# Eddie-Wang1120/Eddie-Wang-Hackathon2023

Hardware: AMD Instinct MI355X
Metric: decode tokens/s, whole job (encoder + cross-KV + language-ID + prefill + greedy decode), Whisper large-v2 int8 weight-only + int8 KV; rtf reported beside it (higher is better)
Workload: dtype f16

## Files before the change

### eddie-wang-hackathon2023_amd/csrc/attn_decode.hip

```cpp
#include <hip/hip_ext.h>

#include <atomic>

#include "common.h"
#include "kernels.h"

namespace wm {

constexpr float ATTN_SCALE = 0.35355339059327373f;
constexpr int MAX_L = 4;

template <bool I8>
__global__ __launch_bounds__(64) void attn_self_kernel(AttnSelfParams p) {
    __builtin_amdgcn_s_setprio(3);

    constexpr int MAXT = 512;
    __shared__ float s_p[MAXT];
    __shared__ h16 s_qall[MAX_L][64], s_knew[MAX_L][64], s_vnew[MAX_L][64];

    const int h = blockIdx.x, lane = threadIdx.x;
    int b = blockIdx.y;
    const int32_t* lsrc = p.live ? p.live : (const int32_t*)p.part;
    const int32_t live_n = lsrc[0], live_b = lsrc[p.live ? 1 + b : 0];
    const int32_t t_now = (p.t_dev ? p.t_dev : (const int32_t*)p.part)[0];
// ... 131 lines not shown
            sum += e;
        }
        sum = wave_sum_nomfma(sum);
        const float inv = 1.0f / sum;
        __syncthreads();
        for (int j = lane; j < nk; j += 64) s_p[j] = r16(s_p[j] * inv);
        __syncthreads();
        float o = 0.f;
        int j = 0;
        if (I8) {
            const int8_t* pv = (const int8_t*)pastV + lane;
#pragma unroll
            for (int u = 0; u < 32; ++u)
                if (u < T) o = fmaf(s_p[u], r16((float)vpre8[u] * t_dq), o);
            j = min(T, 32);
            for (; j + 32 <= T; j += 32) {
                int8_t vq[32];
#pragma unroll
                for (int u = 0; u < 32; ++u) vq[u] = pv[(size_t)(j + u) * 64];
#pragma unroll
                for (int u = 0; u < 32; ++u) o = fmaf(s_p[j + u], r16((float)vq[u] * t_dq), o);
            }
            for (; j + 8 <= T; j += 8) {
                int8_t vq[8];
#pragma unroll
                for (int u = 0; u < 8; ++u) vq[u] = pv[(size_t)(j + u) * 64];
#pragma unroll
                for (int u = 0; u < 8; ++u) o = fmaf(s_p[j + u], r16((float)vq[u] * t_dq), o);
            }
            for (; j < T; ++j) o = fmaf(s_p[j], r16((float)pv[(size_t)j * 64] * t_dq), o);
        } else {
            const h16* pv = (const h16*)pastV + lane;
#pragma unroll
            for (int u = 0; u < 32; ++u)
                if (u < T) o = fmaf(s_p[u], (float)vpre16[u], o);
            j = min(T, 32);
            for (; j + 32 <= T; j += 32) {
                h16 vh[32];
#pragma unroll
                for (int u = 0; u < 32; ++u) vh[u] = pv[(size_t)(j + u) * 64];
#pragma unroll
                for (int u = 0; u < 32; ++u) o = fmaf(s_p[j + u], (float)vh[u], o);
            }
            for (; j + 8 <= T; j += 8) {
                h16 vh[8];
#pragma unroll
                for (int u = 0; u < 8; ++u) vh[u] = pv[(size_t)(j + u) * 64];
#pragma unroll
                for (int u = 0; u < 8; ++u) o = fmaf(s_p[j + u], (float)vh[u], o);
            }
            for (; j < T; ++j) o = fmaf(s_p[j], (float)pv[(size_t)j * 64], o);
        }
        for (; j < nk; ++j) o = fmaf(s_p[j], (float)s_vnew[j - T][lane], o);
        p.out[(size_t)(b * p.L + i) * p.ldo + h * 64 + lane] = (h16)f32_as_is(o);
        __syncthreads();
    }
}

constexpr int SELF_WAVES = 4;
template <bool I8>
__global__ __launch_bounds__(64 * SELF_WAVES) void attn_self_wg_kernel(AttnSelfParams p) {
    __builtin_amdgcn_s_setprio(3);
    constexpr int MAXT = 512;
    constexpr int ES = I8 ? 1 : 2;
    constexpr int ROW_B = 64 * ES;
    constexpr int DIMS = 16 / ES;
    constexpr int NCH = 64 / DIMS;
    constexpr int VROWS = 64 / NCH;
    constexpr int KCH = ROW_B / 16;
    constexpr int VPRE = 4;
    constexpr int NT = 64 * SELF_WAVES;
    __shared__ float s_p[MAXT];
    __shared__ h16 s_qall[MAX_L][64], s_knew[MAX_L][64], s_vnew[MAX_L][64];
    __shared__ float s_o[NT][DIMS + 1];
    __shared__ float s_red[2][SELF_WAVES];
    __shared__ float s_lut[I8 ? 512 + MAX_L * 64 : 1];

    const int h = blockIdx.x, tid = threadIdx.x, lane = tid & 63, wid = tid >> 6;
    int b = blockIdx.y;
    const int32_t* lsrc = p.live ? p.live : (const int32_t*)p.part;
    const int32_t live_n = lsrc[0], live_b = lsrc[p.live ? 1 + b : 0];
    const int32_t t_now = (p.t_dev ? p.t_dev : (const int32_t*)p.part)[0];
    if (p.live) {
        if (b >= live_n) return;
        b = live_b;
    }
    const int T = p.t_dev ? t_now : p.T;
    const int C = p.H * 64;
    const unsigned char* pastK = (const unsigned char*)p.past + ((size_t)b * p.past_bstride + (size_t)(0 * p.H + h) * p.past_cap * 64) * ES;
    const unsigned char* pastV = (const unsigned char*)p.past + ((size_t)b * p.past_bstride + (size_t)(1 * p.H + h) * p.past_cap * 64) * ES;
    const int vr = lane / NCH, vc = lane % NCH;
    uint4 kpre[KCH], vpre[VPRE];
    if (T > 0) {
        const int kr = min(64 * wid + lane, T - 1);
#pragma unroll
        for (int c = 0; c < KCH; ++c) kpre[c] = ((const uint4*)(pastK + (size_t)kr * ROW_B))[c];
#pragma unroll
        for (int n = 0; n < VPRE; ++n) {
            const int row = min((wid + SELF_WAVES * n) * VROWS + vr, T - 1);
            vpre[n] = *(const uint4*)(pastV + (size_t)row * ROW_B + vc * 16);
        }
    }
    const float t_dq = p.kv_scale;
    const float inv_t = 1.0f / p.kv_scale;
    if constexpr (I8) {
        const float d = r16((float)(int)(int8_t)(tid & 255) * t_dq);
// ... 104 lines not shown
        __syncthreads();
        const float inv = 1.0f / ((s_red[1][0] + s_red[1][1]) + (s_red[1][2] + s_red[1][3]));
        if (tid < nk) s_p[tid] = r16(e0 * inv);
        if (tid + NT < nk) s_p[tid + NT] = r16(e1 * inv);
        __syncthreads();
        float o[DIMS];
#pragma unroll
        for (int d = 0; d < DIMS; ++d) o[d] = 0.f;
        auto add_block = [&](int vb, const uint4& w) {
            const int row = vb * VROWS + vr;
            const float pj = row < T ? s_p[row] : 0.f;
            if (I8) {
                const uint32_t ws[4] = {w.x, w.y, w.z, w.w};
#pragma unroll
                for (int d = 0; d < 16; ++d)
                    o[d] = fmaf(pj, s_lut[256 + ((ws[d >> 2] >> (8 * (d & 3))) & 0xff)], o[d]);
            } else {
                const half8v wh = __builtin_bit_cast(half8v, w);
#pragma unroll
                for (int d = 0; d < 8; ++d) o[d] = fmaf(pj, (float)wh[d], o[d]);
            }
        };
#pragma unroll
        for (int n = 0; n < VPRE; ++n) {
            const int vb = wid + SELF_WAVES * n;
            if (vb * VROWS < T) add_block(vb, vpre[n]);
        }
        for (int vb = wid + SELF_WAVES * VPRE; vb * VROWS < T; vb += SELF_WAVES) {
            const int row = min(vb * VROWS + vr, T - 1);
            add_block(vb, *(const uint4*)(pastV + (size_t)row * ROW_B + vc * 16));
        }
#pragma unroll
        for (int d = 0; d < DIMS; ++d) s_o[tid][d] = o[d];
        __syncthreads();
        if (wid == 0) {
            const int ch = lane / DIMS, d = lane % DIMS;
            float part[SELF_WAVES][VROWS];
#pragma unroll
            for (int w = 0; w < SELF_WAVES; ++w)
#pragma unroll
                for (int r = 0; r < VROWS; ++r) part[w][r] = s_o[w * 64 + r * NCH + ch][d];
            float acc = 0.f;
#pragma unroll
            for (int w = 0; w < SELF_WAVES; ++w)
#pragma unroll
                for (int r = 0; r < VROWS; ++r) acc += part[w][r];
            for (int j = T; j < nk; ++j) acc = fmaf(s_p[j], (float)s_vnew[j - T][lane], acc);
            p.out[(size_t)(b * p.L + i) * p.ldo + h * 64 + lane] = (h16)f32_as_is(acc);
        }
        __syncthreads();
    }
}

int launch_attn_self(const AttnSelfParams& p, hipStream_t stream) {
    WM_REQUIRE(p.L >= 1 && p.L <= MAX_L, "attn_self: L=%d out of range [1,%d]", p.L, MAX_L);
    WM_REQUIRE(p.T + p.L <= 512, "attn_self: T+L=%d exceeds 512", p.T + p.L);
    WM_REQUIRE(p.T + p.L <= p.present_cap, "attn_self: present capacity %d < T+L=%d", p.present_cap, p.T + p.L);
    WM_REQUIRE(!p.int8_kv || p.kv_scale > 0.f, "attn_self: int8 KV needs a positive scale");
    WM_REQUIRE(p.waves == 0 || p.waves == 1 || p.waves == SELF_WAVES, "attn_self: waves=%d (0, 1 or %d)", p.waves, SELF_WAVES);
    if (p.waves == SELF_WAVES) {
        if (p.int8_kv) hipLaunchKernelGGL(attn_self_wg_kernel<true>, dim3(p.H, p.B), dim3(64 * SELF_WAVES), 0, stream, p);
        else hipLaunchKernelGGL(attn_self_wg_kernel<false>, dim3(p.H, p.B), dim3(64 * SELF_WAVES), 0, stream, p);
    } else if (p.int8_kv)
        hipLaunchKernelGGL(attn_self_kernel<true>, dim3(p.H, p.B), dim3(64), 0, stream, p);
    else
        hipLaunchKernelGGL(attn_self_kernel<false>, dim3(p.H, p.B), dim3(64), 0, stream, p);
    WM_LAUNCH_CHECK(stream, "attn_self");
    return 0;
}

constexpr int CROSS_MAX_KEYS = 1536;
constexpr int CROSS_MAX_SPLIT = 16;


template <int L, bool I8 = false, int UNR_ = 0, bool SKIP = false>
__global__ __launch_bounds__(256) void attn_cross_kernel(AttnCrossParams p) {
    constexpr int DPL = I8 ? 16 : 8;
    constexpr int LPR = 64 / DPL;
    constexpr int RPI = 64 / LPR;
    constexpr int ESZ = I8 ? 1 : 2;
#ifndef CROSS_UNR
#define CROSS_UNR 4
#endif
    constexpr int UNR = UNR_ > 0 ? UNR_ : CROSS_UNR;
    __shared__ float s_sc[L][CROSS_MAX_KEYS];
    __shared__ float s_red[L][4][2];
    __shared__ float s_o[4][L][64];
    __shared__ unsigned char s_live[SKIP ? CROSS_MAX_KEYS / 8 : 1];

    const int tid = threadIdx.x, lane = tid & 63, wid = __builtin_amdgcn_readfirstlane(tid >> 6);
    const int sub = lane % LPR, rowi = lane / LPR;
    const int per_split = (((p.Tk + p.nsplit - 1) / p.nsplit) + 7) & ~7;
    constexpr int STRIDE = 4 * RPI * UNR;
    const int first = wid * (RPI * UNR);
    const int n_rows = p.live ? p.live[0] : p.B;
    const int n_items = p.H * n_rows * p.nsplit;

    struct Item { int h, b, sp, k_begin, nkeys; const unsigned char* K; const unsigned char* V; };
    auto geometry = [&](int item) {
        Item it;
        it.h = item % p.H; it.b = (item / p.H) % n_rows; it.sp = item / (p.H * n_rows);
        if (p.live) it.b = p.live[1 + it.b];
        it.k_begin = it.sp * per_split;
        it.nkeys = max(0, min(p.Tk, it.k_begin + per_split) - it.k_begin);
        it.K = (const unsigned char*)p.kv + ((size_t)it.b * p.kv_bstride + ((size_t)(0 * p.H + it.h) * p.Tk) * 64) * ESZ;
        it.V = (const unsigned char*)p.kv + ((size_t)it.b * p.kv_bstride + ((size_t)(1 * p.H + it.h) * p.Tk) * 64) * ESZ;
        return it;
    };
    auto issue = [&](u32x4 (&dst)[UNR], const unsigned char* base, int k_begin, int nkeys, int r0) {
#pragma unroll
        for (int u = 0; u < UNR; ++u) {
            const int rr = min(r0 + u * RPI + rowi, nkeys - 1);
            dst[u] = __builtin_nontemporal_load((const u32x4*)(base + ((size_t)(k_begin + rr) * 64 + sub * DPL) * ESZ));
        }
        __builtin_amdgcn_sched_barrier(0);
// ... 395 lines not shown
```

### eddie-wang-hackathon2023_amd/csrc/engine.hip

```cpp
#include <stdarg.h>
#include <stdio.h>
#include <stdlib.h>
#include <string.h>

#include <atomic>
#include <map>
#include <mutex>
#include <unordered_map>
#include <string>
#include <vector>

#include "../../include/whisper_mi355.h"
#include "common.h"
#include "kernels.h"

namespace wm {

static thread_local char g_err[1024] = "";
void set_error(const char* fmt, ...) {
    va_list ap;
    va_start(ap, fmt);
    vsnprintf(g_err, sizeof(g_err), fmt, ap);
    va_end(ap);
}
// ... 1229 lines not shown
}

int wm_argmax(const void* logits, int64_t row_stride, int batch, int n_vocab, int32_t* ids, wm_stream_t stream) {
    WM_REQUIRE(logits && ids && batch >= 1 && n_vocab >= 1, "wm_argmax: null argument or empty input");
    return launch_argmax((const h16*)logits, (long)row_stride, batch, n_vocab, ids, (hipStream_t)stream);
}

int wm_gemm_skinny(const void* A, int lda, int M, int K, const void* Wt, int n_blocks, int w8,
                   const void* scale, int ksplit, float* part, wm_stream_t stream) {
    GemmSkinnyParams p{};
    p.A = (const h16*)A; p.lda = lda; p.M = M; p.K = K; p.Wt = Wt; p.n_blocks = n_blocks; p.w8 = w8;
    p.scale = (const h16*)scale; p.ksplit = ksplit; p.part = part;
    return launch_gemm_skinny(p, (hipStream_t)stream);
}
int wm_gemm_skinny_default_ksplit(int M, int K, int n_blocks, int w8) { return skinny_default_ksplit(M, K, n_blocks, w8); }

int wm_set_rows_path(int min_rows) {
    const int prev = rows_path_min_rows();
    g_rows_min.store(min_rows < 0 ? 0 : min_rows, std::memory_order_relaxed);
    return prev;
}

int wm_gemm_rows(const wm_gemv_io* io, wm_stream_t stream) {
    WM_REQUIRE(io && io->a && io->wt, "wm_gemm_rows: null argument");
    GemvSmallParams p{};
    p.A = (const h16*)io->a; p.lda = io->lda; p.M = io->m; p.K = io->k; p.Wt = io->wt; p.n_blocks = io->n_blocks; p.w8 = io->w8;
    p.scale = (const h16*)io->scale;
    p.ln_g = (const h16*)io->ln_gamma; p.ln_b = (const h16*)io->ln_beta;
    p.mode = io->mode; p.bias = (const h16*)io->bias; p.gelu_kind = io->gelu_kind;
    p.out32 = io->out32; p.ld32 = io->ld32; p.out16 = (h16*)io->out16; p.ld16 = io->ld16; p.n_valid = io->n_valid;
    p.x = (h16*)io->x; p.ldx = io->ldx;
    return launch_gemm_rows(p, (hipStream_t)stream);
}

int wm_lab_knobs(char* buf, size_t cap) {
    std::lock_guard<std::mutex> lk(g_lab_mu);
    if (buf && cap > 0) { strncpy(buf, g_lab_honoured.c_str(), cap - 1); buf[cap - 1] = 0; }
    return (int)g_lab_honoured.size();
}

int wm_set_gemm_small_tiles(int tiles) {
    const int prev = get_gemm_small_tiles();
    set_gemm_small_tiles(tiles);
    return prev;
}

int wm_set_self_attn_waves(int waves) {
    self_attn_waves(1);
    const int prev = g_self_waves.load(std::memory_order_relaxed);
    g_self_waves.store(waves == 1 || waves == 4 ? waves : 0, std::memory_order_relaxed);
    return prev;
}

int wm_set_small_batch_rows(int rows) {
    const int prev = small_path_max_rows();
    g_small_rows.store(rows < 0 ? 0 : (rows > GEMV_SMALL_MAX_M ? GEMV_SMALL_MAX_M : rows), std::memory_order_relaxed);
    return prev;
}

int wm_gemv_fused(const wm_gemv_io* io, wm_stream_t stream) {
    WM_REQUIRE(io && io->a && io->wt, "wm_gemv_fused: null argument");
    GemvSmallParams p{};
    p.A = (const h16*)io->a; p.lda = io->lda; p.M = io->m; p.K = io->k; p.Wt = io->wt; p.n_blocks = io->n_blocks; p.w8 = io->w8;
    p.scale = (const h16*)io->scale;
    p.ln_g = (const h16*)io->ln_gamma; p.ln_b = (const h16*)io->ln_beta;
    p.mode = io->mode; p.bias = (const h16*)io->bias; p.gelu_kind = io->gelu_kind;
    p.out32 = io->out32; p.ld32 = io->ld32; p.out16 = (h16*)io->out16; p.ld16 = io->ld16; p.n_valid = io->n_valid;
    p.x = (h16*)io->x; p.ldx = io->ldx;
    return launch_gemv_small(p, (hipStream_t)stream);
}

int wm_layernorm(const void* x, int ldx, int M, int N, const void* gamma, const void* beta, void* out, int ldo,
                 wm_stream_t stream) {
    return launch_layernorm((const h16*)x, ldx, M, N, (const h16*)gamma, (const h16*)beta, (h16*)out, ldo, (hipStream_t)stream);
}

int wm_attn_encoder(const void* qkv, int ld, int B, int T, int H, void* out, int ldo, wm_stream_t stream) {
    AttnEncParams p{(const h16*)qkv, ld, B, T, H, (h16*)out, ldo};
    return launch_attn_encoder(p, (hipStream_t)stream);
}

int wm_attn_decode_cross(const float* q, int B, int L, int H, int Tk, const void* kv, void* out, int nsplit,
                         float* ws, wm_stream_t stream) {
    AttnCrossParams p{};
    p.part = q; p.ksplit = 1; p.ldp = H * 64; p.bias = nullptr;
    p.B = B; p.L = L; p.H = H; p.Tk = Tk; p.kv = (const h16*)kv; p.kv_bstride = (long)2 * H * Tk * 64;
    p.out = (h16*)out; p.ldo = H * 64; p.nsplit = nsplit; p.ws = ws;
    p.skip_zero_rows = g_cross_v_skip.load(std::memory_order_relaxed);
    return launch_attn_cross(p, (hipStream_t)stream);
}

int wm_set_decode_chain(int on) {
    const int prev = g_decode_chain.load(std::memory_order_relaxed);
    g_decode_chain.store(on < 0 ? DECODE_CHAIN_DEFAULT : (on > 2 ? 2 : on), std::memory_order_relaxed);
    for (ChainDev& cd : g_chain_dev) {
        std::lock_guard<std::mutex> lk(cd.mu);
        if (cd.declined) { cd.declined = false; cd.reason.clear(); }
    }
    return prev;
}

int wm_decode_chain_error(int* out) {
    WM_REQUIRE(out, "wm_decode_chain_error: null argument");
    ChainDev& cd = chain_dev_slot(current_device_index());
    const unsigned v = chain_err_peek(cd);
    *out = (int)v;
// ... 5 lines not shown
    }
    return 0;
}

int wm_decode_chain_status(wm_chain_status* out) {
    WM_REQUIRE(out, "wm_decode_chain_status: null argument");
    ChainDev& cd = chain_dev_slot(current_device_index());
    std::lock_guard<std::mutex> lk(cd.mu);
    memset(out, 0, sizeof(*out));
    out->mode = g_decode_chain.load(std::memory_order_relaxed);
    out->launches = cd.launches.load(std::memory_order_relaxed);
    out->declined_calls = cd.declined_calls.load(std::memory_order_relaxed);
    out->declined = cd.declined ? 1 : 0;
    out->error_pending = chain_err_peek(cd) ? 1 : 0;
    snprintf(out->reason, sizeof(out->reason), "%s", cd.reason.c_str());
    snprintf(out->footprint, sizeof(out->footprint), "%s", cd.footprint.c_str());
    return 0;
}

int wm_debug_occupy(int n_workgroups, size_t lds_bytes, int64_t microseconds, wm_stream_t stream) {
    return launch_occupy(n_workgroups, lds_bytes, (long long)microseconds, (hipStream_t)stream);
}

int wm_set_cross_v_skip(int on) {
    const int prev = g_cross_v_skip.load(std::memory_order_relaxed);
    g_cross_v_skip.store(on < 0 ? CROSS_V_SKIP_DEFAULT : (on ? 1 : 0), std::memory_order_relaxed);
    return prev;
}

int wm_attn_decode_cross_i8(const float* q, int B, int L, int H, int Tk, const void* kv_i8, float kv_scale, void* out, int nsplit,
                            float* ws, wm_stream_t stream) {
    WM_REQUIRE(kv_scale > 0.f, "wm_attn_decode_cross_i8: the scale must be positive");
    AttnCrossParams p{};
    p.part = q; p.ksplit = 1; p.ldp = H * 64; p.bias = nullptr;
    p.B = B; p.L = L; p.H = H; p.Tk = Tk; p.kv = (const h16*)kv_i8; p.kv_bstride = (long)2 * H * Tk * 64;
    p.kv_q8_scale = kv_scale;
    p.out = (h16*)out; p.ldo = H * 64; p.nsplit = nsplit; p.ws = ws;
    return launch_attn_cross(p, (hipStream_t)stream);
}

int wm_attn_decode_self(const float* qkv, int B, int L, int T, int H, const void* past, int past_cap,
                        void* present, int present_cap, int int8_kv, float kv_scale, void* out, wm_stream_t stream) {
    AttnSelfParams p{};
    p.part = qkv; p.ksplit = 1; p.ldp = 3 * H * 64; p.bias = nullptr;
    p.B = B; p.L = L; p.T = T; p.H = H;
    p.present = present; p.present_cap = present_cap; p.present_bstride = (long)2 * H * present_cap * 64;
    if (T > 0 && past) { p.past = past; p.past_cap = past_cap; p.past_bstride = (long)2 * H * past_cap * 64; }
    else { p.past = present; p.past_cap = present_cap; p.past_bstride = p.present_bstride; }
    p.int8_kv = int8_kv; p.kv_scale = kv_scale; p.out = (h16*)out; p.ldo = H * 64;
    p.waves = self_attn_waves(B * L);
    return launch_attn_self(p, (hipStream_t)stream);
}

int wm_quantize_i8(const void* x, void* q, int64_t n, float inv_scale, wm_stream_t stream) {
    return launch_quantize_i8((const h16*)x, (int8_t*)q, (long)n, inv_scale, (hipStream_t)stream);
}

size_t wm_log_mel_workspace_bytes(int batch, int n_samples, int n_mels) {
    return log_mel_workspace_bytes(batch, n_samples, n_mels);
}

int wm_log_mel(const float* audio, int batch, int n_samples, int64_t audio_ld, const float* filters, int n_mels,
               void* mel_f16, float* mel_f32, void* workspace, size_t workspace_bytes, wm_stream_t stream) {
    return launch_log_mel(audio, batch, n_samples, (long)audio_ld, filters, n_mels, (h16*)mel_f16, mel_f32, workspace,
                          workspace_bytes, (hipStream_t)stream);
}

}
```

### eddie-wang-hackathon2023_amd/csrc/kernels.h

```cpp
#pragma once
#include "common.h"

namespace wm {

struct GemmBigParams {
    const h16* A; int lda; int M; int K;
    const void* W; int N;
    const h16* bias;
    h16* C; int ldc;
    const h16* residual; int ldr; int res_mod;
    int act;
    int colscale_n; float colscale;
    int out_mode;
    int hs_T, hs_H, hs_kv;
    float q8_inv_scale;
    int a_rows; long a_bstride;
    int c_rows; long c_bstride;
    int max_wgs;
    int nt_flags;
    int tile_rows;
};
int launch_gemm_f16(const GemmBigParams& p, hipStream_t stream);
constexpr int GEMM_SMALL_TILES_DEFAULT = 150;
constexpr int GEMM_TINY_TILES_DEFAULT = 160;
// ... 74 lines not shown
    const float* part; int ksplit; int M; int N; int ldp;
    long part_sstride;
    const h16* bias;
    int mode; int gelu_kind;
    h16* x; int ldx;
    const h16* ln_g; const h16* ln_b;
    h16* out; int ldo;
    int eager;
};
int launch_row_finish(const RowFinishParams& p, hipStream_t stream);

struct EmbedParams {
    const int32_t* tokens; int tokens_ld;
    int M;
    int L;
    const void* emb_tiles; int C;
    const h16* pos;
    h16* x; int ldx;
    int n_vocab;
    const int32_t* t_dev;
    unsigned* generation;
};
int launch_embed(const EmbedParams& p, hipStream_t stream);

int launch_mel_transpose_pad(const h16* mel, int B, int n_mels, int T, h16* out ,
                             hipStream_t stream);
int launch_zero_pad_rows(h16* buf, int B, int Tpad, int C, hipStream_t stream);
int launch_layernorm(const h16* x, int ldx, int M, int N, const h16* g, const h16* b, h16* out, int ldo,
                     hipStream_t stream);

struct AttnEncParams {
    const h16* qkv; int ld;
    int B, T, H;
    h16* out; int ldo;
    int max_wgs;
};
int launch_attn_encoder(const AttnEncParams& p, hipStream_t stream);

struct AttnSelfParams {
    const float* part; int ksplit; int ldp;
    long part_sstride;
    const h16* bias;
    int B, L, T, H;
    const void* past; long past_bstride; int past_cap;
    void* present; long present_bstride; int present_cap;
    int int8_kv; float kv_scale;
    float* amax;
    const int32_t* t_dev;
    h16* out; int ldo;
    const int32_t* live;
    int waves;
};
int launch_attn_self(const AttnSelfParams& p, hipStream_t stream);

struct AttnCrossParams {
    const float* part; int ksplit; int ldp;
    long part_sstride;
    const h16* bias;
    int B, L, H, Tk;
    const h16* kv; long kv_bstride;
    float kv_q8_scale;
    h16* out; int ldo;
    int nsplit;
    float* ws;
    const int32_t* live;
    int skip_zero_rows;
};
constexpr int CROSS_V_SKIP_DEFAULT = 1;
int launch_attn_cross(const AttnCrossParams& p, hipStream_t stream, hipEvent_t ev_start = nullptr, hipEvent_t ev_stop = nullptr);

struct GreedyParams {
    h16* logits; long ld_row;
    int B; int V;
    int32_t* tokens; int ld_tok; int cur_len;
    float* sum_logprobs;
    const int32_t* suppress; int n_suppress;
    const int32_t* blank; int n_blank;
    int sample_begin; int eot; int timestamp_begin; int max_initial_ts;
    int apply_rules;
    int32_t* n_done;
    const int32_t* t_dev;
    int32_t* done;
    const int32_t* row_limit;
    float temperature;
    uint32_t seed_lo, seed_hi; const uint32_t* seed_dev;
    int row0;
};
int launch_greedy(const GreedyParams& p, hipStream_t stream);
int launch_step_advance(int32_t* counter, hipStream_t stream);
int launch_step_finish(int32_t* counter, const int32_t* done, int B, int32_t* live, hipStream_t stream);
int launch_argmax(const h16* logits, long ld_row, int B, int V, int32_t* ids, hipStream_t stream);

constexpr int BEAM_MAX = 8, BEAM_POOL_MAX = 16;
struct BeamCand { float lp; int32_t tok; };
struct BeamParams {
    GreedyParams g;
    int K, max_cand, ignore_eot;
    int32_t* parent;
    int32_t* fin_tokens; float* fin_scores; int32_t* fin_len; int32_t* fin_count;
    int32_t* live_len;
    BeamCand* cand;
};
int launch_beam_step(const BeamParams& p, hipStream_t stream);
struct KvReorderParams {
    void* const* layers; int n_layer, rows, K, H, cap, elem_bytes;
    const int32_t* parent; const int32_t* done; int n_last; const int32_t* t_dev;
// ... 11 lines not shown
```

### eddie-wang-hackathon2023_amd/native.py

```python
from __future__ import annotations

import atexit
import ctypes as C
import os
from typing import Optional, Sequence

import sys
import warnings


def _hip_already_initialised() -> bool:
    t = sys.modules.get("torch")
    try:
        return bool(t is not None and t.cuda.is_initialized())
    except Exception:
        return False


def _configure_runtime() -> dict:
    name = "DEBUG_CLR_GRAPH_PACKET_CAPTURE"
    late = _hip_already_initialised()
    if name in os.environ:
        return {"name": name, "value": os.environ[name], "set_by": "caller", "in_time": None}
    if os.environ.get("WM_GRAPH_NODE_REPLAY", "1") == "0":
        return {"name": name, "value": None, "set_by": "nobody (WM_GRAPH_NODE_REPLAY=0)", "in_time": None}
    os.environ[name] = "0"
    if late:
        warnings.warn("whisper_mi355: the HIP runtime was initialised before this package was imported, so "
                      f"{name}=0 (node-by-node graph replay, 6-10 % of the small-batch token step) is NOT in effect: "
                      "import the package before the first torch.cuda call, or export the variable yourself", RuntimeWarning, stacklevel=3)
    return {"name": name, "value": "0", "set_by": "package", "in_time": not late}


RUNTIME_KNOBS = _configure_runtime()


def runtime_report() -> dict:
    rep = dict(RUNTIME_KNOBS)
    rep["effective_env"] = os.environ.get(RUNTIME_KNOBS["name"])
    if _lib is not None:
        buf = C.create_string_buffer(4096)
        _lib.wm_lab_knobs(buf, 4096)
        rep["lab_knobs_honoured"] = buf.value.decode() or None
    return rep


_HERE = os.path.dirname(os.path.abspath(__file__))
LIB_PATH = os.environ.get("WM_LIBRARY_PATH") or os.path.join(_HERE, "libwhisper_mi355.so")

EXPORTS = (
    "wm_version", "wm_last_error", "wm_device_count", "wm_engine_create", "wm_engine_destroy",
    "wm_engine_info", "wm_engine_weight_bytes", "wm_encoder_workspace_bytes", "wm_encoder_forward",
    "wm_encoder_forward_shared", "wm_encoder_forward_range",
    "wm_cross_kv_workspace_bytes", "wm_cross_kv", "wm_decoder_workspace_bytes", "wm_decoder_step",
    "wm_greedy_step", "wm_gemm", "wm_gemm_skinny", "wm_gemm_skinny_default_ksplit", "wm_layernorm",
    "wm_attn_encoder", "wm_attn_decode_cross", "wm_attn_decode_self", "wm_quantize_i8",
    "wm_profile_configure", "wm_profile_read", "wm_step_advance", "wm_log_mel_workspace_bytes", "wm_log_mel",
    "wm_flac_info", "wm_flac_decode", "wm_conv1d_gelu", "wm_argmax", "wm_gemv_fused", "wm_gemm_rows", "wm_set_rows_path", "wm_set_small_batch_rows", "wm_set_self_attn_waves", "wm_set_gemm_small_tiles", "wm_lab_knobs", "wm_set_cross_v_skip", "wm_set_decode_chain", "wm_decode_chain_error", "wm_decode_chain_status", "wm_debug_occupy", "wm_decoder_step_multi", "wm_stream_create_cu_mask", "wm_stream_destroy", "wm_attn_decode_cross_i8", "wm_debug_timeline",
    "wm_step_finish",
    "wm_beam_workspace_bytes", "wm_beam_step", "wm_kv_reorder",
    "wm_gemm_ex", "wm_row_finish", "wm_embed", "wm_mel_transpose_pad", "wm_zero_pad_rows",
)


ABI_VERSION = 8

import threading as _threading
CAPTURE_LOCK = _threading.RLock()


class WmError(RuntimeError):
    pass


class WmFlacStreamInfo(C.Structure):
    _fields_ = [("sample_rate", C.c_int32), ("channels", C.c_int32), ("bits_per_sample", C.c_int32),
                ("max_block_size", C.c_int32), ("total_samples", C.c_int64), ("md5", C.c_uint8 * 16)]


class WmChainStatus(C.Structure):
    _fields_ = [("mode", C.c_int32), ("declined", C.c_int32), ("error_pending", C.c_int32), ("pad_", C.c_int32),
                ("launches", C.c_int64), ("declined_calls", C.c_int64), ("reason", C.c_char * 200), ("footprint", C.c_char * 200)]


def chain_status() -> dict:
    st = WmChainStatus()
    check(load_library().wm_decode_chain_status(C.byref(st)), "wm_decode_chain_status")
    return {"mode": st.mode, "declined": bool(st.declined), "error_pending": bool(st.error_pending), "launches": int(st.launches),
            "declined_calls": int(st.declined_calls), "reason": st.reason.decode(), "footprint": st.footprint.decode()}


class WmDims(C.Structure):
    _fields_ = [(n, C.c_int32) for n in (
        "n_mels", "n_audio_ctx", "n_audio_state", "n_audio_head", "n_audio_layer",
        "n_vocab", "n_text_ctx", "n_text_state", "n_text_head", "n_text_layer")]

    def to_dict(self):
        return {n: int(getattr(self, n)) for n, _ in self._fields_}


class WmDecoderIO(C.Structure):
    _fields_ = [
        ("batch", C.c_int32), ("n_new", C.c_int32), ("n_past", C.c_int32),
        ("tokens", C.c_void_p), ("tokens_ld", C.c_int32), ("positional_embedding", C.c_void_p),
        ("past", C.POINTER(C.c_void_p)), ("past_capacity", C.c_int32),
        ("present", C.POINTER(C.c_void_p)), ("present_capacity", C.c_int32),
        ("cross", C.POINTER(C.c_void_p)),
        ("logits", C.c_void_p),
        ("workspace", C.c_void_p), ("workspace_bytes", C.c_size_t),
        ("qkv_amax", C.c_void_p),
        ("n_past_dev", C.c_void_p),
# ... 84 lines not shown
        ("x", C.c_void_p), ("ldx", C.c_int32),
        ("ln_gamma", C.c_void_p), ("ln_beta", C.c_void_p),
        ("out", C.c_void_p), ("ldo", C.c_int32),
    ]


_lib: Optional[C.CDLL] = None


def load_library(path: str = LIB_PATH) -> C.CDLL:
    global _lib
    if _lib is not None:
        return _lib
    if not os.path.exists(path):
        raise WmError(f"{path} not found: build it with `python __graft_entry__.py` "
                      f"(hipcc --offload-arch=gfx950); there is no fallback path")
    lib = C.CDLL(path, mode=C.RTLD_GLOBAL)
    for name in EXPORTS:
        if not hasattr(lib, name):
            raise WmError(f"{path} does not export {name}")
    vp, i32, sz = C.c_void_p, C.c_int, C.c_size_t
    lib.wm_version.restype = i32
    if lib.wm_version() != ABI_VERSION:
        raise WmError(f"{path} has ABI version {lib.wm_version()}, this binding needs {ABI_VERSION}: rebuild it "
                      f"(python __graft_entry__.py)")
    lib.wm_last_error.restype = C.c_char_p
    lib.wm_device_count.argtypes = [C.POINTER(i32)]
    lib.wm_engine_create.argtypes = [vp, sz, i32, C.POINTER(vp)]
    lib.wm_engine_destroy.argtypes = [vp]
    lib.wm_engine_destroy.restype = None
    lib.wm_engine_info.argtypes = [vp, C.POINTER(C.c_int32), C.POINTER(C.c_uint32), C.POINTER(WmDims)]
    lib.wm_engine_weight_bytes.argtypes = [vp]
    lib.wm_engine_weight_bytes.restype = sz
    lib.wm_encoder_workspace_bytes.argtypes = [vp, i32]
    lib.wm_encoder_workspace_bytes.restype = sz
    lib.wm_encoder_forward.argtypes = [vp, vp, i32, vp, vp, sz, vp]
    lib.wm_encoder_forward_shared.argtypes = [vp, vp, i32, vp, vp, sz, i32, vp]
    lib.wm_encoder_forward_range.argtypes = [vp, vp, i32, vp, vp, sz, i32, i32, i32, vp]
    lib.wm_cross_kv_workspace_bytes.argtypes = [vp, i32]
    lib.wm_cross_kv_workspace_bytes.restype = sz
    lib.wm_cross_kv.argtypes = [vp, vp, i32, C.POINTER(vp), vp, sz, vp]
    lib.wm_decoder_workspace_bytes.argtypes = [vp, i32, i32]
    lib.wm_decoder_workspace_bytes.restype = sz
    lib.wm_decoder_step.argtypes = [vp, C.POINTER(WmDecoderIO), vp]
    lib.wm_greedy_step.argtypes = [C.POINTER(WmGreedyIO), vp]
    lib.wm_gemm.argtypes = [vp, i32, i32, i32, vp, i32, i32, vp, vp, vp, i32, i32, vp, i32, vp, sz, vp]
    lib.wm_conv1d_gelu.argtypes = [vp, i32, i32, i32, vp, i32, vp, i32, i32, i32, vp, vp]
    lib.wm_argmax.argtypes = [vp, C.c_int64, i32, i32, vp, vp]
    lib.wm_gemv_fused.argtypes = [C.POINTER(WmGemvIO), vp]
    lib.wm_set_small_batch_rows.argtypes = [i32]
    lib.wm_gemm_rows.argtypes = [C.POINTER(WmGemvIO), vp]
    lib.wm_set_rows_path.argtypes = [i32]
    lib.wm_set_self_attn_waves.argtypes = [i32]
    lib.wm_set_gemm_small_tiles.argtypes = [i32]
    lib.wm_lab_knobs.argtypes = [C.c_char_p, sz]
    lib.wm_set_cross_v_skip.argtypes = [i32]
    lib.wm_set_decode_chain.argtypes = [i32]
    lib.wm_decode_chain_error.argtypes = [C.POINTER(C.c_int)]
    lib.wm_decode_chain_status.argtypes = [C.POINTER(WmChainStatus)]
    lib.wm_debug_occupy.argtypes = [i32, sz, C.c_int64, vp]
    lib.wm_gemm_skinny.argtypes = [vp, i32, i32, i32, vp, i32, i32, vp, i32, vp, vp]
    lib.wm_gemm_skinny_default_ksplit.argtypes = [i32, i32, i32, i32]
    lib.wm_layernorm.argtypes = [vp, i32, i32, i32, vp, vp, vp, i32, vp]
    lib.wm_attn_encoder.argtypes = [vp, i32, i32, i32, i32, vp, i32, vp]
    lib.wm_attn_decode_cross.argtypes = [vp, i32, i32, i32, i32, vp, vp, i32, vp, vp]
    lib.wm_attn_decode_self.argtypes = [vp, i32, i32, i32, i32, vp, i32, vp, i32, i32, C.c_float, vp, vp]
    lib.wm_quantize_i8.argtypes = [vp, vp, C.c_int64, C.c_float, vp]
    lib.wm_log_mel_workspace_bytes.argtypes = [i32, i32, i32]
    lib.wm_log_mel_workspace_bytes.restype = sz
    lib.wm_log_mel.argtypes = [vp, i32, i32, C.c_int64, vp, i32, vp, vp, vp, sz, vp]
    lib.wm_decoder_step_multi.argtypes = [vp, i32, C.POINTER(C.POINTER(WmDecoderIO)), C.POINTER(vp), vp]
    lib.wm_stream_create_cu_mask.argtypes = [C.POINTER(C.c_uint32), i32, C.POINTER(vp)]
    lib.wm_stream_destroy.argtypes = [vp]
    lib.wm_attn_decode_cross_i8.argtypes = [vp, i32, i32, i32, i32, vp, C.c_float, vp, i32, vp, vp]
    lib.wm_flac_info.argtypes = [vp, sz, C.POINTER(WmFlacStreamInfo)]
    lib.wm_flac_decode.argtypes = [vp, sz, vp, C.c_int64, C.POINTER(C.c_int64)]
    lib.wm_step_advance.argtypes = [vp, vp]
    lib.wm_step_finish.argtypes = [vp, vp, i32, vp, vp]
    lib.wm_beam_workspace_bytes.argtypes = [i32, i32]
    lib.wm_beam_workspace_bytes.restype = sz
    lib.wm_beam_step.argtypes = [C.POINTER(WmBeamIO), vp]
    lib.wm_kv_reorder.argtypes = [vp, i32, i32, i32, i32, i32, i32, vp, vp, i32, vp, vp]
    lib.wm_debug_timeline.argtypes = [vp, i32]
    lib.wm_gemm_ex.argtypes = [C.POINTER(WmGemmIO), vp]
    lib.wm_row_finish.argtypes = [C.POINTER(WmRowFinishIO), vp]
    lib.wm_embed.argtypes = [vp, i32, i32, i32, vp, i32, vp, vp, i32, i32, vp, vp, vp]
    lib.wm_mel_transpose_pad.argtypes = [vp, i32, i32, i32, vp, vp]
    lib.wm_zero_pad_rows.argtypes = [vp, i32, i32, i32, vp]
    lib.wm_profile_configure.argtypes = [i32, i32, i32]
    lib.wm_profile_read.argtypes = [C.POINTER(C.c_double), C.POINTER(C.c_int64), i32]
    _lib = lib
    return lib


def check(rc: int, what: str = ""):
    if rc != 0:
        msg = load_library().wm_last_error().decode(errors="replace")
        raise WmError(f"{what or 'libwhisper_mi355'} failed (rc={rc}): {msg}")


def ptr_array(tensors: Sequence) -> "C.Array":
    arr = (C.c_void_p * len(tensors))()
    for i, t in enumerate(tensors):
        arr[i] = None if t is None else (t.data_ptr() if hasattr(t, "data_ptr") else int(t))
    return arr

# ... 64 lines not shown
```

### include/whisper_mi355.h

```cpp
#ifndef WHISPER_MI355_H
#define WHISPER_MI355_H

#include <stddef.h>
#include <stdint.h>

#ifdef __cplusplus
extern "C" {
#endif

typedef struct wm_engine wm_engine;
typedef void* wm_stream_t;

enum { WM_ENGINE_ENCODER = 0, WM_ENGINE_DECODER = 1, WM_ENGINE_CROSS_KV = 2 };
enum { WM_FLAG_WEIGHT_ONLY_INT8 = 1, WM_FLAG_INT8_KV = 2, WM_FLAG_GELU_TANH = 4,
       WM_FLAG_INT8_CROSS_KV = 16  };

typedef struct wm_dims {
    int32_t n_mels, n_audio_ctx, n_audio_state, n_audio_head, n_audio_layer;
    int32_t n_vocab, n_text_ctx, n_text_state, n_text_head, n_text_layer;
} wm_dims;

#define WM_ABI_VERSION 8
int wm_version(void);
const char* wm_last_error(void);
// ... 88 lines not shown
                  const int32_t* parent, const int32_t* done, int n_last, const int32_t* n_past_dev, wm_stream_t stream);

int wm_gemm(const void* A, int lda, int M, int K, const void* W, int N, int w8, const void* scale,
            const void* bias, const void* residual, int ldr, int act, void* C, int ldc,
            void* workspace, size_t workspace_bytes, wm_stream_t stream);
int wm_conv1d_gelu(const void* x_pad, int B, int T_in, int C_in, const void* W, int K, const void* bias,
                   int C_out, int stride, int gelu, void* out, wm_stream_t stream);
typedef struct wm_gemm_io {
    const void* a; int32_t lda, m, k;
    const void* w; int32_t n;
    const void* bias;
    void* c; int32_t ldc;
    const void* residual; int32_t ldr, res_mod;
    int32_t act;
    int32_t colscale_n; float colscale;
    int32_t out_mode, hs_t, hs_h, hs_kv;
    float q8_inv_scale;
    int32_t a_rows; int64_t a_bstride;
    int32_t c_rows; int64_t c_bstride;
    int32_t max_wgs, tile_rows;
} wm_gemm_io;
int wm_gemm_ex(const wm_gemm_io* io, wm_stream_t stream);
typedef struct wm_row_finish_io {
    const float* part; int32_t ksplit, m, n, ldp; int64_t part_sstride;
    const void* bias;
    int32_t mode, gelu_kind;
    void* x; int32_t ldx;
    const void* ln_gamma; const void* ln_beta;
    void* out; int32_t ldo;
} wm_row_finish_io;
int wm_row_finish(const wm_row_finish_io* io, wm_stream_t stream);
int wm_embed(const int32_t* tokens, int tokens_ld, int M, int L, const void* emb_tiles, int C, const void* pos,
             void* x, int ldx, int n_vocab, const int32_t* t_dev, uint32_t* generation, wm_stream_t stream);
int wm_mel_transpose_pad(const void* mel, int B, int n_mels, int T, void* out, wm_stream_t stream);
int wm_zero_pad_rows(void* buf, int B, int Tpad, int C, wm_stream_t stream);
int wm_argmax(const void* logits, int64_t row_stride, int batch, int n_vocab, int32_t* ids, wm_stream_t stream);
int wm_gemm_skinny(const void* A, int lda, int M, int K, const void* Wt, int n_blocks, int w8,
                   const void* scale, int ksplit, float* part, wm_stream_t stream);
int wm_gemm_skinny_default_ksplit(int M, int K, int n_blocks, int w8);
typedef struct wm_gemv_io {
    const void* a; int32_t lda, m, k;
    const void* wt; int32_t n_blocks, w8; const void* scale;
    const void* ln_gamma; const void* ln_beta;
    int32_t mode; const void* bias; int32_t gelu_kind;
    float* out32; int32_t ld32;
    void* out16; int32_t ld16, n_valid;
    void* x; int32_t ldx;
} wm_gemv_io;
int wm_gemv_fused(const wm_gemv_io* io, wm_stream_t stream);
int wm_set_small_batch_rows(int rows);
int wm_gemm_rows(const wm_gemv_io* io, wm_stream_t stream);
int wm_set_rows_path(int min_rows);
int wm_set_self_attn_waves(int waves);
int wm_set_gemm_small_tiles(int tiles);
typedef struct wm_chain_status {
    int32_t mode;
    int32_t declined;
    int32_t error_pending;
    int32_t pad_;
    int64_t launches;
    int64_t declined_calls;
    char reason[200];
    char footprint[200];
} wm_chain_status;
int wm_set_decode_chain(int on);
int wm_decode_chain_error(int* out);
int wm_decode_chain_status(wm_chain_status* out);
int wm_debug_occupy(int n_workgroups, size_t lds_bytes, int64_t microseconds, wm_stream_t stream);
int wm_set_cross_v_skip(int on);
int wm_lab_knobs(char* buf, size_t cap);
int wm_layernorm(const void* x, int ldx, int M, int N, const void* gamma, const void* beta,
                 void* out, int ldo, wm_stream_t stream);
int wm_attn_encoder(const void* qkv, int ld, int B, int T, int H, void* out, int ldo, wm_stream_t stream);
int wm_attn_decode_cross(const float* q, int B, int L, int H, int Tk, const void* kv, void* out,
                         int nsplit, float* ws, wm_stream_t stream);
int wm_attn_decode_cross_i8(const float* q, int B, int L, int H, int Tk, const void* kv_i8, float kv_scale,
                            void* out, int nsplit, float* ws, wm_stream_t stream);
int wm_attn_decode_self(const float* qkv, int B, int L, int T, int H, const void* past, int past_cap,
                        void* present, int present_cap, int int8_kv, float kv_scale, void* out,
                        wm_stream_t stream);
int wm_quantize_i8(const void* x, void* q, int64_t n, float inv_scale, wm_stream_t stream);

size_t wm_log_mel_workspace_bytes(int batch, int n_samples, int n_mels);
int wm_log_mel(const float* audio, int batch, int n_samples, int64_t audio_ld, const float* filters,
               int n_mels, void* mel_f16, float* mel_f32, void* workspace, size_t workspace_bytes,
               wm_stream_t stream);

typedef struct wm_flac_streaminfo {
    int32_t sample_rate;
    int32_t channels;
    int32_t bits_per_sample;
    int32_t max_block_size;
    int64_t total_samples;
    uint8_t md5[16];
} wm_flac_streaminfo;
int wm_flac_info(const void* data, size_t bytes, wm_flac_streaminfo* info);
int wm_flac_decode(const void* data, size_t bytes, int32_t* pcm, int64_t capacity_samples,
                   int64_t* n_decoded);

int wm_profile_configure(int enabled, int layer_stride, int max_samples);
int wm_profile_read(double* total_ms, int64_t* count, int reset);
int wm_debug_timeline(void* buf, int capacity);

#ifdef __cplusplus
}
#endif
#endif
```

Measured before the change: 16600.

## Add single-wave self-attention kernel that prefetches K into registers and streams V via LDS

Adds a new single-wave decode self-attention kernel that issues K-row prefetches into registers and asynchronous global-to-LDS loads of V chunks before the QKV reduction and KV write. Later blocks use a double-buffered ring, so the memory latency of the past KV cache overlaps with compute. It is enabled by default, behind a runtime toggle, whenever the 4-wave path is not selected. It also adds an extended API entry point exposing ksplit, bias, device T and live rows. In exchange it uses more LDS and registers per workgroup and relies on hand-placed waitcnt ordering, which could limit occupancy or be fragile.

```diff
diff --git a/eddie-wang-hackathon2023_amd/csrc/attn_decode.hip b/eddie-wang-hackathon2023_amd/csrc/attn_decode.hip
--- a/eddie-wang-hackathon2023_amd/csrc/attn_decode.hip
+++ b/eddie-wang-hackathon2023_amd/csrc/attn_decode.hip
@@ -207,6 +207,231 @@
             for (; j < T; ++j) o = fmaf(s_p[j], (float)pv[(size_t)j * 64], o);
         }
         for (; j < nk; ++j) o = fmaf(s_p[j], (float)s_vnew[j - T][lane], o);
+        p.out[(size_t)(b * p.L + i) * p.ldo + h * 64 + lane] = (h16)f32_as_is(o);
+        __syncthreads();
+    }
+}
+
+constexpr int SELF_VP = 5;
+template <bool I8>
+__global__ __launch_bounds__(64) void attn_self_one_trip_kernel(AttnSelfParams p) {
+    __builtin_amdgcn_s_setprio(3);
+
+    constexpr int MAXT = 512;
+    constexpr int ES = I8 ? 1 : 2;
+    constexpr int ROW_B = 64 * ES;
+    constexpr int KCH = ROW_B / 16;
+    constexpr int KPRE = I8 ? 3 : 2;
+    constexpr int RPP = 64 / KCH;
+    constexpr int VP = SELF_VP;
+    constexpr int VCH = VP * RPP;
+    __shared__ float s_p[MAXT];
+    __shared__ h16 s_qall[MAX_L][64], s_knew[MAX_L][64], s_vnew[MAX_L][64];
+    __shared__ __attribute__((aligned(16))) unsigned char s_v[2][VP * 1024];
+
+    const int h = blockIdx.x, lane = threadIdx.x;
+    int b = blockIdx.y;
+    const int32_t* lsrc = p.live ? p.live : (const int32_t*)p.part;
+    const int32_t live_n = lsrc[0], live_b = lsrc[p.live ? 1 + b : 0];
+    const int32_t t_now = (p.t_dev ? p.t_dev : (const int32_t*)p.part)[0];
+    if (p.live) {
+        if (b >= live_n) return;
+        b = live_b;
+    }
+    const int T = p.t_dev ? t_now : p.T;
+    const int C = p.H * 64;
+    const unsigned char* pastK = (const unsigned char*)p.past + ((size_t)b * p.past_bstride + (size_t)(0 * p.H + h) * p.past_cap * 64) * ES;
+    const unsigned char* pastV = (const unsigned char*)p.past + ((size_t)b * p.past_bstride + (size_t)(1 * p.H + h) * p.past_cap * 64) * ES;
+    const int nch = (T + VCH - 1) / VCH;
+    const bool ring = nch > 2;
+
+    uint4 kpre0[KCH], kpre1[KCH], kpre2[KCH];
+    auto k_load = [&](uint4 (&dst)[KCH], int blk) {
+        const uint4* src = (const uint4*)(pastK + (uint32_t)(min(blk * 64 + lane, T - 1) * ROW_B));
+#pragma unroll
+        for (int c = 0; c < KCH; ++c) dst[c] = src[c];
+    };
+    auto v_issue = [&](int c, bool whole) {
+        unsigned char* dst = s_v[c & 1];
+#pragma unroll
+        for (int u = 0; u < VP; ++u) {
+            const int r0 = (c * VP + u) * RPP;
+            if (whole || r0 < T) {
+                const int row = min(r0 + lane / KCH, T - 1);
+                __builtin_amdgcn_global_load_lds((const __attribute__((address_space(1))) void*)(pastV + (uint32_t)(row * ROW_B + (lane % KCH) * 16)),
+                                                 (__attribute__((address_space(3))) void*)(dst + u * 1024), 16, 0, 0);
+            }
+        }
+    };
+    if (T > 0) {
+        k_load(kpre0, 0);
+        if (T > 64) k_load(kpre1, 1);
+        if (KPRE > 2 && T > 128) k_load(kpre2, 2);
+        v_issue(0, ring);
+        if (nch > 1) v_issue(1, ring);
+    }
+    const float t_dq = p.kv_scale;
+    const float inv_t = 1.0f / p.kv_scale;
+    const size_t sstride = p.part_sstride ? (size_t)p.part_sstride : (size_t)p.B * p.L * p.ldp;
+
+    for (int i = 0; i < p.L; ++i) {
+        const int m = b * p.L + i;
+        float q = 0.f, k = 0.f, v = 0.f;
+        const h16* bsrc = p.bias ? p.bias + h * 64 : (const h16*)p.part;
+        const int bstep = p.bias ? C : 0;
+        const h16 bq_raw = bsrc[lane], bk_raw = (bsrc + bstep)[lane], bv_raw = (bsrc + 2 * bstep)[lane];
+        {
+            const float* row = p.part + (size_t)m * p.ldp + h * 64;
+            int s = 0;
+            for (; s + 4 <= p.ksplit; s += 4) {
+                const float* r0 = row + (size_t)s * sstride;
+                const float* r1 = r0 + sstride; const float* r2 = r1 + sstride; const float* r3 = r2 + sstride;
+                const float q0 = r0[lane], q1 = r1[lane], q2 = r2[lane], q3 = r3[lane];
+                const float k0 = (r0 + C)[lane], k1 = (r1 + C)[lane], k2 = (r2 + C)[lane], k3 = (r3 + C)[lane];
+                const float v0 = (r0 + 2 * C)[lane], v1 = (r1 + 2 * C)[lane], v2 = (r2 + 2 * C)[lane], v3 = (r3 + 2 * C)[lane];
+                q += (q0 + q1) + (q2 + q3); k += (k0 + k1) + (k2 + k3); v += (v0 + v1) + (v2 + v3);
+            }
+            for (; s < p.ksplit; ++s) {
+                const float* r0 = row + (size_t)s * sstride;
+                q += r0[lane]; k += (r0 + C)[lane]; v += (r0 + 2 * C)[lane];
+            }
+        }
+        q = r16(q + (p.bias ? (float)bq_raw : 0.f));
+        k = r16(k + (p.bias ? (float)bk_raw : 0.f));
+        v = r16(v + (p.bias ? (float)bv_raw : 0.f));
+        if (p.amax) {
+            const float a = wave_max_nomfma(fmaxf(fabsf(q), fmaxf(fabsf(k), fabsf(v))));
+            if (lane == 0) atomicMax((unsigned int*)p.amax, __float_as_uint(a));
+        }
+        s_knew[i][lane] = (h16)k;
+        s_vnew[i][lane] = (h16)v;
+        const size_t off_k = (size_t)b * p.present_bstride + ((size_t)(0 * p.H + h) * p.present_cap + T + i) * 64 + lane;
+        const size_t off_v = (size_t)b * p.present_bstride + ((size_t)(1 * p.H + h) * p.present_cap + T + i) * 64 + lane;
+        if (I8) {
+            ((int8_t*)p.present)[off_k] = (int8_t)fminf(127.f, fmaxf(-128.f, rintf(k * inv_t)));
+            ((int8_t*)p.present)[off_v] = (int8_t)fminf(127.f, fmaxf(-128.f, rintf(v * inv_t)));
+        } else {
+            ((h16*)p.present)[off_k] = (h16)k;
+            ((h16*)p.present)[off_v] = (h16)v;
+        }
+        s_qall[i][lane] = (h16)r16(q * ATTN_SCALE);
+    }
+    const bool inplace = (p.past == p.present) && (p.past_cap == p.present_cap) && (p.past_bstride == p.present_bstride);
+    if (!inplace && T > 0) {
+        for (int kv = 0; kv < 2; ++kv) {
+            const unsigned char* src = (const unsigned char*)p.past + ((size_t)b * p.past_bstride + (size_t)(kv * p.H + h) * p.past_cap * 64) * ES;
+            unsigned char* dst = (unsigned char*)p.present + ((size_t)b * p.present_bstride + (size_t)(kv * p.H + h) * p.present_cap * 64) * ES;
+            const int n16 = T * 64 * ES / 16;
+            for (int c = lane; c < n16; c += 64) ((uint4*)dst)[c] = ((const uint4*)src)[c];
+        }
+    }
+    asm volatile("s_waitcnt vmcnt(0)" ::: "memory");
+    __syncthreads();
+
+    for (int i = 0; i < p.L; ++i) {
+        const h16* s_q = s_qall[i];
+        const int nk = T + i + 1;
+        if (i > 0 && T > 0) {
+            k_load(kpre0, 0);
+            if (T > 64) k_load(kpre1, 1);
+            if (KPRE > 2 && T > 128) k_load(kpre2, 2);
+        }
+        if (i > 0 && ring) {
+            asm volatile("s_waitcnt lgkmcnt(0)" ::: "memory");
+            v_issue(0, true);
+            v_issue(1, true);
+        }
+        float mx = -INFINITY;
+#pragma unroll 1
+        for (int blk = 0; blk * 64 < nk; ++blk) {
+            const int j0 = blk * 64;
+            asm volatile("" ::: "memory");
+            const uint4 (&kc)[KCH] = kpre0;
+            const int j = j0 + lane;
+            float sc = -INFINITY;
+            if (j < nk) {
+                float acc = 0.f;
+                if (j < T) {
+                    if (I8) {
+#pragma unroll
+                        for (int c = 0; c < 4; ++c) {
+                            const uint4 w = kc[c];
+                            const uint32_t ws[4] = {w.x, w.y, w.z, w.w};
+#pragma unroll
+                            for (int e = 0; e < 16; ++e) {
+                                const int8_t q8 = (int8_t)((ws[e >> 2] >> (8 * (e & 3))) & 0xff);
+                                const float kd = r16(r16((float)q8 * t_dq) * ATTN_SCALE);
+                                acc = fmaf((float)s_q[c * 16 + e], kd, acc);
+                            }
+                            __builtin_amdgcn_sched_barrier(0);
+                        }
+                    } else {
+#pragma unroll
+                        for (int c = 0; c < 8; ++c) {
+                            const half8v w = __builtin_bit_cast(half8v, kc[c % KCH]);
+#pragma unroll
+                            for (int e = 0; e < 8; ++e)
+                                acc = fmaf((float)s_q[c * 8 + e], r16((float)w[e] * ATTN_SCALE), acc);
+                            __builtin_amdgcn_sched_barrier(0);
+                        }
+                    }
+                } else {
+                    const h16* kn = s_knew[j - T];
+#pragma unroll 8
+                    for (int e = 0; e < 64; ++e) acc = fmaf((float)s_q[e], r16((float)kn[e] * ATTN_SCALE), acc);
+                }
+                sc = r16(f32_as_is(acc));
+            }
+            if (j < MAXT) s_p[j] = sc;
+            mx = fmaxf(mx, sc);
+#pragma unroll
+            for (int c = 0; c < KCH; ++c) {
+                kpre0[c] = kpre1[c];
+                if (KPRE > 2) kpre1[c] = kpre2[c];
+            }
+            if ((blk + KPRE) * 64 < T) k_load(KPRE > 2 ? kpre2 : kpre1, blk + KPRE);
+        }
+        mx = wave_max_nomfma(mx);
+        float sum = 0.f;
+        __syncthreads();
+        for (int j = lane; j < nk; j += 64) {
+            const float e = __expf(s_p[j] - mx);
+            s_p[j] = e;
+            sum += e;
+        }
+        sum = wave_sum_nomfma(sum);
+        const float inv = 1.0f / sum;
+        __syncthreads();
+        for (int j = lane; j < nk; j += 64) s_p[j] = r16(s_p[j] * inv);
+        __syncthreads();
+        float o = 0.f;
+        for (int c = 0; c < nch; ++c) {
+            if (ring) {
+                if (c + 1 < nch) asm volatile("s_waitcnt vmcnt(%0)" :: "n"(VP) : "memory");
+                else asm volatile("s_waitcnt vmcnt(0)" ::: "memory");
+            }
+            const unsigned char* vb = s_v[c & 1] + lane * ES;
+            const float* pc = s_p + c * VCH;
+            const int nr = min(T - c * VCH, VCH);
+            auto val = [&](int r) -> float {
+                if constexpr (I8) return r16((float)((const int8_t*)vb)[r * ROW_B] * t_dq);
+                else return (float)*(const h16*)(vb + r * ROW_B);
+            };
+            int r = 0;
+            for (; r + 8 <= nr; r += 8) {
+                float x[8];
+#pragma unroll
+                for (int u = 0; u < 8; ++u) x[u] = val(r + u);
+#pragma unroll
+                for (int u = 0; u < 8; ++u) o = fmaf(pc[r + u], x[u], o);
+            }
+            for (; r < nr; ++r) o = fmaf(pc[r], val(r), o);
+            if (ring && c + 2 < nch) {
+                asm volatile("s_waitcnt lgkmcnt(0)" ::: "memory");
+                v_issue(c + 2, true);
+            }
+        }
+        for (int j = T; j < nk; ++j) o = fmaf(s_p[j], (float)s_vnew[j - T][lane], o);
         p.out[(size_t)(b * p.L + i) * p.ldo + h * 64 + lane] = (h16)f32_as_is(o);
         __syncthreads();
     }
@@ -417,6 +642,17 @@
     }
 }
 
+std::atomic<int> g_self_one_trip{-1};
+int get_attn_self_one_trip() {
+    int v = g_self_one_trip.load(std::memory_order_relaxed);
+    if (v < 0) {
+        v = lab_env_int("WM_SELF_ONE_TRIP", ATTN_SELF_ONE_TRIP_DEFAULT) ? 1 : 0;
+        g_self_one_trip.store(v, std::memory_order_relaxed);
+    }
+    return v;
+}
+void set_attn_self_one_trip(int on) { g_self_one_trip.store(on < 0 ? ATTN_SELF_ONE_TRIP_DEFAULT : (on ? 1 : 0), std::memory_order_relaxed); }
+
 int launch_attn_self(const AttnSelfParams& p, hipStream_t stream) {
     WM_REQUIRE(p.L >= 1 && p.L <= MAX_L, "attn_self: L=%d out of range [1,%d]", p.L, MAX_L);
     WM_REQUIRE(p.T + p.L <= 512, "attn_self: T+L=%d exceeds 512", p.T + p.L);
@@ -426,6 +662,9 @@
     if (p.waves == SELF_WAVES) {
         if (p.int8_kv) hipLaunchKernelGGL(attn_self_wg_kernel<true>, dim3(p.H, p.B), dim3(64 * SELF_WAVES), 0, stream, p);
         else hipLaunchKernelGGL(attn_self_wg_kernel<false>, dim3(p.H, p.B), dim3(64 * SELF_WAVES), 0, stream, p);
+    } else if (get_attn_self_one_trip()) {
+        if (p.int8_kv) hipLaunchKernelGGL(attn_self_one_trip_kernel<true>, dim3(p.H, p.B), dim3(64), 0, stream, p);
+        else hipLaunchKernelGGL(attn_self_one_trip_kernel<false>, dim3(p.H, p.B), dim3(64), 0, stream, p);
     } else if (p.int8_kv)
         hipLaunchKernelGGL(attn_self_kernel<true>, dim3(p.H, p.B), dim3(64), 0, stream, p);
     else
diff --git a/eddie-wang-hackathon2023_amd/csrc/engine.hip b/eddie-wang-hackathon2023_amd/csrc/engine.hip
--- a/eddie-wang-hackathon2023_amd/csrc/engine.hip
+++ b/eddie-wang-hackathon2023_amd/csrc/engine.hip
@@ -1305,6 +1305,12 @@
     return prev;
 }
 
+int wm_set_self_attn_one_trip(int on) {
+    const int prev = get_attn_self_one_trip();
+    set_attn_self_one_trip(on);
+    return prev;
+}
+
 int wm_set_small_batch_rows(int rows) {
     const int prev = small_path_max_rows();
     g_small_rows.store(rows < 0 ? 0 : (rows > GEMV_SMALL_MAX_M ? GEMV_SMALL_MAX_M : rows), std::memory_order_relaxed);
@@ -1416,6 +1422,22 @@
     return launch_attn_self(p, (hipStream_t)stream);
 }
 
+int wm_attn_decode_self_ex(const float* qkv, int ksplit, int64_t slab_stride, const void* bias, int B, int L, int T, int H,
+                           const void* past, int past_cap, void* present, int present_cap, int int8_kv, float kv_scale,
+                           const int32_t* t_dev, const int32_t* live_rows, void* out, wm_stream_t stream) {
+    WM_REQUIRE(qkv && present && out && ksplit >= 1, "wm_attn_decode_self_ex: null argument or ksplit < 1");
+    AttnSelfParams p{};
+    p.part = qkv; p.ksplit = ksplit; p.ldp = 3 * H * 64; p.part_sstride = (long)slab_stride; p.bias = (const h16*)bias;
+    p.B = B; p.L = L; p.T = T; p.H = H;
+    p.present = present; p.present_cap = present_cap; p.present_bstride = (long)2 * H * present_cap * 64;
+    if (past) { p.past = past; p.past_cap = past_cap; p.past_bstride = (long)2 * H * past_cap * 64; }
+    else { p.past = present; p.past_cap = present_cap; p.past_bstride = p.present_bstride; }
+    p.int8_kv = int8_kv; p.kv_scale = kv_scale; p.out = (h16*)out; p.ldo = H * 64;
+    p.t_dev = t_dev; p.live = live_rows;
+    p.waves = self_attn_waves(B * L);
+    return launch_attn_self(p, (hipStream_t)stream);
+}
+
 int wm_quantize_i8(const void* x, void* q, int64_t n, float inv_scale, wm_stream_t stream) {
     return launch_quantize_i8((const h16*)x, (int8_t*)q, (long)n, inv_scale, (hipStream_t)stream);
 }
diff --git a/eddie-wang-hackathon2023_amd/csrc/kernels.h b/eddie-wang-hackathon2023_amd/csrc/kernels.h
--- a/eddie-wang-hackathon2023_amd/csrc/kernels.h
+++ b/eddie-wang-hackathon2023_amd/csrc/kernels.h
@@ -150,6 +150,9 @@
     int waves;
 };
 int launch_attn_self(const AttnSelfParams& p, hipStream_t stream);
+constexpr int ATTN_SELF_ONE_TRIP_DEFAULT = 1;
+void set_attn_self_one_trip(int on);
+int get_attn_self_one_trip();
 
 struct AttnCrossParams {
     const float* part; int ksplit; int ldp;
diff --git a/eddie-wang-hackathon2023_amd/native.py b/eddie-wang-hackathon2023_amd/native.py
--- a/eddie-wang-hackathon2023_amd/native.py
+++ b/eddie-wang-hackathon2023_amd/native.py
@@ -56,7 +56,7 @@
     "wm_greedy_step", "wm_gemm", "wm_gemm_skinny", "wm_gemm_skinny_default_ksplit", "wm_layernorm",
     "wm_attn_encoder", "wm_attn_decode_cross", "wm_attn_decode_self", "wm_quantize_i8",
     "wm_profile_configure", "wm_profile_read", "wm_step_advance", "wm_log_mel_workspace_bytes", "wm_log_mel",
-    "wm_flac_info", "wm_flac_decode", "wm_conv1d_gelu", "wm_argmax", "wm_gemv_fused", "wm_gemm_rows", "wm_set_rows_path", "wm_set_small_batch_rows", "wm_set_self_attn_waves", "wm_set_gemm_small_tiles", "wm_lab_knobs", "wm_set_cross_v_skip", "wm_set_decode_chain", "wm_decode_chain_error", "wm_decode_chain_status", "wm_debug_occupy", "wm_decoder_step_multi", "wm_stream_create_cu_mask", "wm_stream_destroy", "wm_attn_decode_cross_i8", "wm_debug_timeline",
+    "wm_flac_info", "wm_flac_decode", "wm_conv1d_gelu", "wm_argmax", "wm_gemv_fused", "wm_gemm_rows", "wm_set_rows_path", "wm_set_small_batch_rows", "wm_set_self_attn_waves", "wm_set_self_attn_one_trip", "wm_attn_decode_self_ex", "wm_set_gemm_small_tiles", "wm_lab_knobs", "wm_set_cross_v_skip", "wm_set_decode_chain", "wm_decode_chain_error", "wm_decode_chain_status", "wm_debug_occupy", "wm_decoder_step_multi", "wm_stream_create_cu_mask", "wm_stream_destroy", "wm_attn_decode_cross_i8", "wm_debug_timeline",
     "wm_step_finish",
     "wm_beam_workspace_bytes", "wm_beam_step", "wm_kv_reorder",
     "wm_gemm_ex", "wm_row_finish", "wm_embed", "wm_mel_transpose_pad", "wm_zero_pad_rows",
@@ -247,6 +247,8 @@
     lib.wm_gemm_rows.argtypes = [C.POINTER(WmGemvIO), vp]
     lib.wm_set_rows_path.argtypes = [i32]
     lib.wm_set_self_attn_waves.argtypes = [i32]
+    lib.wm_set_self_attn_one_trip.argtypes = [i32]
+    lib.wm_attn_decode_self_ex.argtypes = [vp, i32, C.c_int64, vp, i32, i32, i32, i32, vp, i32, vp, i32, i32, C.c_float, vp, vp, vp, vp]
     lib.wm_set_gemm_small_tiles.argtypes = [i32]
     lib.wm_lab_knobs.argtypes = [C.c_char_p, sz]
     lib.wm_set_cross_v_skip.argtypes = [i32]
diff --git a/include/whisper_mi355.h b/include/whisper_mi355.h
--- a/include/whisper_mi355.h
+++ b/include/whisper_mi355.h
@@ -164,6 +164,7 @@
 int wm_gemm_rows(const wm_gemv_io* io, wm_stream_t stream);
 int wm_set_rows_path(int min_rows);
 int wm_set_self_attn_waves(int waves);
+int wm_set_self_attn_one_trip(int on);
 int wm_set_gemm_small_tiles(int tiles);
 typedef struct wm_chain_status {
     int32_t mode;
@@ -191,6 +192,9 @@
 int wm_attn_decode_self(const float* qkv, int B, int L, int T, int H, const void* past, int past_cap,
                         void* present, int present_cap, int int8_kv, float kv_scale, void* out,
                         wm_stream_t stream);
+int wm_attn_decode_self_ex(const float* qkv, int ksplit, int64_t slab_stride, const void* bias, int B, int L, int T, int H,
+                           const void* past, int past_cap, void* present, int present_cap, int int8_kv, float kv_scale,
+                           const int32_t* t_dev, const int32_t* live_rows, void* out, wm_stream_t stream);
 int wm_quantize_i8(const void* x, void* q, int64_t n, float inv_scale, wm_stream_t stream);
 
 size_t wm_log_mel_workspace_bytes(int batch, int n_samples, int n_mels);
```

New measurement: 16610 (median of 2 runs). About the same (+0.1%).
